# itailang/SampleNet

Measured on AMD Instinct MI355X. Metric: point-clouds/sec fwd+bwd, Bx1024->64 soft-proj+Chamfer, higher is better.
Workload: dtype f32; 1 GPU; BASELINE configs[1]: SampleNet sampler train step (fwd + simplification/projection losses + bwd), B=32 per GPU, 1024->64 points, K=8, bottleneck 128; no optimizer step; batch_per_gpu=32, global_batch=32, n_in=1024, n_out=64, group_size=8, parallelism=dp1, rccl_ranks=0, grad_allreduce=none, execution=whole step replayed as one hipGraph

## Files before the change

samplenet_amd/csrc/geometry_ops.hip:

```cpp
#include <algorithm>
#include <cstdlib>
#include <cstring>

#include "sn_common.h"
#include "step_tail.h"

#pragma clang fp contract(off)

namespace sn {

struct sn_xyz3 {
    float x, y, z;
};

constexpr int kMaxPrefixes = 16;

struct ImplicitGrad {
    const float *gL;
    const int *argmax_t, *argmax_s;
    float ct, cmax_t, cs, cmax_s;
    float gscale = 1.f;
};

__global__ void __launch_bounds__(256) chamfer_bwd_kernel(int nt, int ns, const float *__restrict__ T,
                                                          const float *__restrict__ S,
                                                          const float *__restrict__ gT,
                                                          const int *__restrict__ idxT,
                                                          const float *__restrict__ gS,
                                                          const int *__restrict__ idxS, float *__restrict__ gradT,
                                                          int own_first, ImplicitGrad ig, int t_layout)
{
    const int lane = threadIdx.x & 63;
    const int wave = __builtin_amdgcn_readfirstlane(threadIdx.x >> 6);
    const int nwaves = blockDim.x >> 6;
    const int b = blockIdx.x;
    T += (size_t)b * nt * 3, S += (size_t)b * ns * 3;
    idxT += (size_t)b * nt, idxS += (size_t)b * ns;
    const bool implicit = ig.gL != nullptr;
    float gLv = 0.f;
    int amt = -1, ams = -1;
    if (implicit) {
        gLv = *ig.gL * ig.gscale;
        if (ig.argmax_t) amt = ig.argmax_t[b];
        if (ig.argmax_s) ams = ig.argmax_s[b];
    } else {
        gT += (size_t)b * nt, gS += (size_t)b * ns;
    }
    gradT += (size_t)b * nt * 3;
    for (int j = blockIdx.y * nwaves + wave; j < nt; j += gridDim.y * nwaves) {
        const int o0 = t_layout ? j : j * 3, os = t_layout ? nt : 1;
        const float tx = T[o0], ty = T[o0 + os], tz = T[o0 + 2 * os];
        const int j2 = idxT[j];
        const float g = (implicit ? gLv * (ig.ct + (j == amt ? ig.cmax_t : 0.f)) : gT[j]) * 2;
        const float ox = g * (tx - S[j2 * 3 + 0]);
        const float oy = g * (ty - S[j2 * 3 + 1]);
        const float oz = g * (tz - S[j2 * 3 + 2]);
        float ax = 0.f, ay = 0.f, az = 0.f;
        if (own_first) ax += ox, ay += oy, az += oz;
        for (int l0 = 0; l0 < ns; l0 += 64 * 8) {
            int is[8];
#pragma unroll
            for (int q = 0; q < 8; ++q) {
                const int l = l0 + q * 64 + lane;
                is[q] = idxS[l < ns ? l : 0];
            }
#pragma unroll
            for (int q = 0; q < 8; ++q) {
                const int l = l0 + q * 64 + lane;
                sn_u64 mask = __ballot(l < ns && is[q] == j);
                while (mask) {
                    const int ll = l0 + q * 64 + __builtin_ctzll(mask);
                    mask &= mask - 1;
                    const float gg = (implicit ? gLv * (ig.cs + (ll == ams ? ig.cmax_s : 0.f)) : gS[ll]) * 2;
                    ax -= gg * (S[ll * 3 + 0] - tx);
                    ay -= gg * (S[ll * 3 + 1] - ty);
                    az -= gg * (S[ll * 3 + 2] - tz);
                }
            }
        }
        if (!own_first) ax += ox, ay += oy, az += oz;
        if (lane < 3) gradT[o0 + lane * os] = lane == 0 ? ax : (lane == 1 ? ay : az);
    }
}

template <int PPL>
__global__ void __launch_bounds__(256) chamfer_bwd_reg_kernel(int nt, int ns, const float *__restrict__ T,
                                                              const float *__restrict__ S,
                                                              const float *__restrict__ gT,
                                                              const int *__restrict__ idxT,
                                                              const float *__restrict__ gS,
                                                              const int *__restrict__ idxS, float *__restrict__ gradT,
                                                              int own_first, ImplicitGrad ig, int t_layout)
{
    const int lane = threadIdx.x & 63;
    const int wave = __builtin_amdgcn_readfirstlane(threadIdx.x >> 6);
    const int nwaves = blockDim.x >> 6;
    const int b = blockIdx.x;
    T += (size_t)b * nt * 3, S += (size_t)b * ns * 3;
    idxT += (size_t)b * nt, idxS += (size_t)b * ns;
    const bool implicit = ig.gL != nullptr;
    float gLv = 0.f;
    int amt = -1, ams = -1;
    if (implicit) {
        gLv = *ig.gL * ig.gscale;
        if (ig.argmax_t) amt = ig.argmax_t[b];
        if (ig.argmax_s) ams = ig.argmax_s[b];
    } else {
        gT += (size_t)b * nt, gS += (size_t)b * ns;
    }
    gradT += (size_t)b * nt * 3;

    float sx[PPL], sy[PPL], sz[PPL], gg[PPL];
    int is[PPL];
#pragma unroll
    for (int i = 0; i < PPL; ++i) {
        const int l = i * 64 + lane;
        const int lc = l < ns ? l : 0;
        const sn_xyz3 sv = *reinterpret_cast<const sn_xyz3 *>(S + (size_t)lc * 3);
        sx[i] = sv.x, sy[i] = sv.y, sz[i] = sv.z;
        is[i] = l < ns ? idxS[lc] : -1;
        gg[i] = (implicit ? gLv * (ig.cs + (l == ams ? ig.cmax_s : 0.f)) : gS[lc]) * 2;
    }
    for (int j = blockIdx.y * nwaves + wave; j < nt; j += gridDim.y * nwaves) {
        const int o0 = t_layout ? j : j * 3, os = t_layout ? nt : 1;
        const float tx = T[o0], ty = T[o0 + os], tz = T[o0 + 2 * os];
        const int j2 = idxT[j];
        const float g = (implicit ? gLv * (ig.ct + (j == amt ? ig.cmax_t : 0.f)) : gT[j]) * 2;
        const float ox = g * (tx - S[j2 * 3 + 0]);
        const float oy = g * (ty - S[j2 * 3 + 1]);
        const float oz = g * (tz - S[j2 * 3 + 2]);
        float ax = 0.f, ay = 0.f, az = 0.f;
        if (own_first) ax += ox, ay += oy, az += oz;
#pragma unroll
        for (int i = 0; i < PPL; ++i) {
            sn_u64 mask = __ballot(is[i] == j);
            if (mask) {
                const float cx = gg[i] * (sx[i] - tx), cy = gg[i] * (sy[i] - ty), cz = gg[i] * (sz[i] - tz);
                while (mask) {
                    const int t = __builtin_ctzll(mask);
                    mask &= mask - 1;
                    ax -= readlane_f(cx, t);
                    ay -= readlane_f(cy, t);
                    az -= readlane_f(cz, t);
                }
            }
        }
        if (!own_first) ax += ox, ay += oy, az += oz;
        if (lane < 3) gradT[o0 + lane * os] = lane == 0 ? ax : (lane == 1 ? ay : az);
    }
}

static const int kChamferBwdGroups = 1024;

static void launch_chamfer_bwd(int b, int ysplit, int nt, int ns, const float *T, const float *S, const float *gT,
                               const int *idxT, const float *gS, const int *idxS, float *gradT, int own_first,
                               const ImplicitGrad &ig, hipStream_t st, int t_layout = 0)
{
    const dim3 grid(b, ysplit), block(256);
#define SN_CB(PPL_) \
    hipLaunchKernelGGL(chamfer_bwd_reg_kernel<PPL_>, grid, block, 0, st, nt, ns, T, S, gT, idxT, gS, idxS, gradT, own_first, ig, t_layout)
    if (ns <= 64) SN_CB(1);
    else if (ns <= 256) SN_CB(4);
    else if (ns <= 1024) SN_CB(16);
    else if (ns <= 2048) SN_CB(32);
    else
        hipLaunchKernelGGL(chamfer_bwd_kernel, grid, block, 0, st, nt, ns, T, S, gT, idxT, gS, idxS, gradT, own_first, ig, t_layout);
#undef SN_CB
}

struct SoftBwdArgs {
    const float *P;
    const float *Q;
    const int *idx;
    const float *temperature;
    float min_sigma;
    int p_layout, q_layout;
    int n, m, k;
    const float *grad_proj;
    int gproj_layout;
    const float *weights_in;
    const float *grad_weights;
    float *grad_Q;
    int gq_layout;
    float *grad_P;
    float *gp_contrib;
    float *grad_sigma_partial;
    const float *gconst;
    float gconst_div;
    int accumulate_q;
};

struct SoftQuery {
    float qx, qy, qz;
    int id;
    float gx, gy, gz;
    float go0, go1, go2;
};

__device__ __forceinline__ float dpp_row_shr1(float x)
{
    return __int_as_float(__builtin_amdgcn_update_dpp(0, __float_as_int(x), 0x111, 0xf, 0xf, true));
}
__device__ __forceinline__ float dpp_row_shr1_self(float x)
{
    return __int_as_float(__builtin_amdgcn_update_dpp(__float_as_int(x), __float_as_int(x), 0x111, 0xf, 0xf, false));
}

__device__ __forceinline__ void soft_bwd_load_index(const SoftBwdArgs &a, int b, int j, int lane, const float *__restrict__ Qb,
                                                    SoftQuery &q)
{
    const int m = a.m, K = a.k;
    q.qx = Qb[pt_off(a.q_layout, m, j, 0)];
    q.qy = Qb[pt_off(a.q_layout, m, j, 1)];
    q.qz = Qb[pt_off(a.q_layout, m, j, 2)];
    const int sub = K <= 16 ? (lane & 15) : lane;
    q.id = sub < K ? a.idx[((size_t)b * m + j) * K + sub] : 0;
    q.go0 = q.go1 = q.go2 = 0.f;
    if (a.grad_proj) {
        const float *gp = a.grad_proj + (size_t)b * 3 * m;
        q.go0 = gp[pt_off(a.gproj_layout, m, j, 0)];
        q.go1 = gp[pt_off(a.gproj_layout, m, j, 1)];
        q.go2 = gp[pt_off(a.gproj_layout, m, j, 2)];
    }
}

__device__ __forceinline__ void soft_bwd_load_points(const SoftBwdArgs &a, int lane, const float *__restrict__ Pb, SoftQuery &q)
{
    const int n = a.n, K = a.k;
    const int sub = K <= 16 ? (lane & 15) : lane;
    q.gx = q.gy = q.gz = 0.f;
    if (sub < K) {
        q.gx = Pb[pt_off(a.p_layout, n, q.id, 0)];
        q.gy = Pb[pt_off(a.p_layout, n, q.id, 1)];
        q.gz = Pb[pt_off(a.p_layout, n, q.id, 2)];
    }
}

template <bool FUSED>
__device__ __forceinline__ void soft_bwd_math(const SoftBwdArgs &a, int b, int j, int lane, float sigma, const SoftQuery &q,
                                              float &aqx_o, float &aqy_o, float &aqz_o, float &asg_o)
{
    const int n = a.n, m = a.m, K = a.k;
    const bool rows = K <= 16;
    const int sub = rows ? (lane & 15) : lane;
    const bool act = sub < K;
    const int id = q.id;
    const float gx = q.gx, gy = q.gy, gz = q.gz;
    const float dx = gx - q.qx, dy = gy - q.qy, dz = gz - q.qz;
    const float d = (dx * dx + dy * dy) + dz * dz;
    const float s = act ? -(d / sigma) : -INFINITY;
    float mx, den;
    if (rows) {
        mx = s;
        for (int t = 1; t < K; ++t) mx = fmaxf(s, dpp_row_shr1_self(mx));
        mx = readlane_f(mx, K - 1);
    } else {
        mx = readlane_f(s, 0);
        for (int t = 1; t < K; ++t) mx = fmaxf(mx, readlane_f(s, t));
    }
    const float e = act ? expf(s - mx) : 0.f;
    if (rows) {
        den = e;
        for (int t = 1; t < K; ++t) den = e + dpp_row_shr1(den);
        den = readlane_f(den, K - 1);
    } else {
        den = 0.f;
        for (int t = 0; t < K; ++t) den += readlane_f(e, t);
    }
    const float w = e / den;

    float gw;
    float go0 = 0.f, go1 = 0.f, go2 = 0.f;
    if (FUSED) {
        if (a.grad_proj) {
            go0 = q.go0, go1 = q.go1, go2 = q.go2;
        } else {
            go0 = go1 = go2 = *a.gconst / a.gconst_div;
        }
        gw = (go0 * gx + go1 * gy) + go2 * gz;
    } else {
        gw = act ? a.grad_weights[((size_t)b * m + j) * K + sub] : 0.f;
    }
    float dot;
    if (rows) {
        const float wg = w * gw;
        dot = wg;
        for (int t = 1; t < K; ++t) dot = wg + dpp_row_shr1(dot);
        dot = readlane_f(dot, K - 1);
    } else {
        dot = 0.f;
        for (int t = 0; t < K; ++t) dot += readlane_f(w, t) * readlane_f(gw, t);
    }
    const float gs = act ? w * (gw - dot) : 0.f;
    const float gd = -gs / sigma;
    const float cx = 2.0f * gd * dx, cy = 2.0f * gd * dy, cz = 2.0f * gd * dz;
    const float sg = act ? gs * d / (sigma * sigma) : 0.f;
    float aqx = 0.f, aqy = 0.f, aqz = 0.f, asg = 0.f;
    if (rows) {
        const int row = lane >> 4;
// ... 124 lines not shown

__global__ void __launch_bounds__(256) weighted_gather_bwd_kernel(int c, int n, int m, int K,
                                                                  const float *__restrict__ X,
                                                                  const int *__restrict__ idx,
                                                                  const float *__restrict__ w,
                                                                  const float *__restrict__ go,
                                                                  float *__restrict__ gw, float *__restrict__ gX,
                                                                  float *__restrict__ contrib = nullptr)
{
    const int b = blockIdx.y;
    const size_t e = (size_t)blockIdx.x * blockDim.x + threadIdx.x;
    if (e >= (size_t)m * K) return;
    const int j = (int)(e / K);
    const int id = idx[(size_t)b * m * K + e];
    const float wt = w[(size_t)b * m * K + e];
    float acc = 0.f;
    for (int ch = 0; ch < c; ++ch) {
        const float g = go[((size_t)b * c + ch) * m + j];
        acc += g * X[((size_t)b * c + ch) * n + id];
        if (contrib) contrib[((size_t)b * c + ch) * m * K + e] = g * wt;
        else if (gX) atomicAdd(&gX[((size_t)b * c + ch) * n + id], g * wt);
    }
    if (gw) gw[(size_t)b * m * K + e] = acc;
}

__global__ void __launch_bounds__(256) group_point_kernel(int n, int c, int m, int ns, const float *__restrict__ points,
                                                          const int *__restrict__ idx, float *__restrict__ out)
{
    const int b = blockIdx.y;
    const size_t tot = (size_t)m * ns * c;
    for (size_t e = (size_t)blockIdx.x * blockDim.x + threadIdx.x; e < tot; e += (size_t)gridDim.x * blockDim.x) {
        const int l = (int)(e % c);
        const size_t jk = e / c;
        const int ii = idx[(size_t)b * m * ns + jk];
        out[(size_t)b * tot + e] = points[((size_t)b * n + ii) * c + l];
    }
}

template <bool CHANNEL_MAJOR>
__global__ void __launch_bounds__(256) index_add_ordered_kernel(int n, int c, int ne, const int *__restrict__ idx,
                                                                const float *__restrict__ src, float *__restrict__ dst)
{
    const int b = blockIdx.y, lane = threadIdx.x & 63;
    const int row0 = blockIdx.x * 256 + (threadIdx.x & ~63);
    const int row = row0 + lane;
    const bool live = row < n;
    idx += (size_t)b * ne;
    src += (size_t)b * ne * c;
    dst += (size_t)b * n * c;
    auto d = [&](int l) -> float & { return dst[CHANNEL_MAJOR ? (size_t)l * n + row : (size_t)row * c + l]; };
    if (live)
        for (int l = 0; l < c; ++l) d(l) = 0.f;
    for (int e0 = 0; e0 < ne; e0 += 64) {
        const int mine = e0 + lane < ne ? idx[e0 + lane] : -1;
        sn_u64 hits = __ballot((unsigned)(mine - row0) < 64u);
        while (hits) {
            const int t = __builtin_ctzll(hits);
            hits &= hits - 1;
            const int id = __builtin_amdgcn_readlane(mine, t), e = e0 + t;
            if (live && id == row)
                for (int l = 0; l < c; ++l) d(l) += src[CHANNEL_MAJOR ? (size_t)l * ne + e : (size_t)e * c + l];
        }
    }
}

constexpr long long kIndexAddOrderedWork = 1ll << 26;
template <bool CHANNEL_MAJOR>
__global__ void __launch_bounds__(256) index_add_atomic_kernel(int n, int c, long long ne, const int *__restrict__ idx,
                                                               const float *__restrict__ src, float *__restrict__ dst)
{
    const int b = blockIdx.y;
    idx += (size_t)b * ne;
    src += (size_t)b * ne * c;
    dst += (size_t)b * n * c;
    const size_t tot = (size_t)ne * c;
    for (size_t t = (size_t)blockIdx.x * blockDim.x + threadIdx.x; t < tot; t += (size_t)gridDim.x * blockDim.x) {
        const size_t e = CHANNEL_MAJOR ? t % (size_t)ne : t / c;
        const int l = (int)(CHANNEL_MAJOR ? t / (size_t)ne : t % c);
        const int row = idx[e];
        if ((unsigned)row < (unsigned)n) atomicAdd(&dst[CHANNEL_MAJOR ? (size_t)l * n + row : (size_t)row * c + l], src[t]);
    }
}

__global__ void __launch_bounds__(256) grouping_operation_kernel(int c, int n, int m, int ns,
                                                                 const float *__restrict__ feat,
                                                                 const int *__restrict__ idx, float *__restrict__ out)
{
    const int b = blockIdx.y;
    const size_t mk = (size_t)m * ns, tot = (size_t)c * mk;
    for (size_t e = (size_t)blockIdx.x * blockDim.x + threadIdx.x; e < tot; e += (size_t)gridDim.x * blockDim.x) {
        const int ch = (int)(e / mk);
        const size_t jk = e % mk;
        const int ii = idx[(size_t)b * mk + jk];
        out[(size_t)b * tot + e] = feat[((size_t)b * c + ch) * n + ii];
    }
}

static inline unsigned grid_for(size_t tot, int block = 256, unsigned cap = 4096)
{
    size_t g = (tot + block - 1) / block;
    return (unsigned)(g < 1 ? 1 : (g > cap ? cap : g));
}

}

using namespace sn;

struct StepLossFinal {
    int B, M, N, nproj;
    float w, alpha, lmbda, min_sigma;
    const float *part;
    const float *temperature;
    float *loss;
};

__device__ __forceinline__ void step_loss_final(const StepLossFinal &f, int t)
{
    float s1 = 0.f, mx = 0.f, s2 = 0.f, sp = 0.f;
    for (int b = t; b < f.B; b += 64) s1 += f.part[b * 4], mx += f.part[b * 4 + 1], s2 += f.part[b * 4 + 2], sp += f.part[b * 4 + 3];
    const float T = *f.temperature;
#pragma unroll
    for (int o = 32; o > 0; o >>= 1) {
        s1 += __shfl_xor(s1, o);
        mx += __shfl_xor(mx, o);
        s2 += __shfl_xor(s2, o);
        sp += __shfl_xor(sp, o);
    }
    if (t != 0) return;
    const float c12 = s1 / ((float)f.B * (float)f.M), cmax = mx / (float)f.B, c21 = s2 / ((float)f.B * (float)f.N);
    const float lsimp = c12 + cmax + f.w * c21;
    f.loss[0] = f.alpha * lsimp + f.lmbda * sn_sigma(T, f.min_sigma) + sp / ((float)f.B * (float)f.nproj);
    f.loss[1] = lsimp;
}

struct StepLossFold {
    int G;
    const sn_u64 *keys;
    const sn_u64 *qmax;
    float *dpsum;
};


#ifdef SN_CS_TIMELINE
__device__ unsigned long long g_cs_tl[8192 * 16];
#define CS_TL(slot)                                                                                              \
    do {                                                                                                         \
        if (threadIdx.x == 0) g_cs_tl[((blockIdx.y * gridDim.x + blockIdx.x) & 8191) * 16 + (slot)] = wall_clock64(); \
    } while (0)
#if SN_CS_TIMELINE >= 2
#define CS_TL_DRAIN() asm volatile("s_waitcnt vmcnt(0) lgkmcnt(0)" ::: "memory")
#else
#define CS_TL_DRAIN()
#endif
#else
#define CS_TL(slot)
#define CS_TL_DRAIN()
#endif

template <int PPL>
__global__ void __launch_bounds__(256) chamfer_soft_bwd_kernel(int nt, int ns, const float *__restrict__ T,
                                                               const float *__restrict__ S, const int *__restrict__ idxT,
                                                               const int *__restrict__ idxS, float *__restrict__ gradT,
                                                               ImplicitGrad ig, SoftBwdArgs sa, StepLossFinal fin,
                                                               StepLossFold fold)
{
    __shared__ float s_part[4];
    __shared__ int s_ip[PPL * 64];
    __shared__ float s_red[3][4];
    __shared__ int s_am;
    const int lane = threadIdx.x & 63;
    const int wave = __builtin_amdgcn_readfirstlane(threadIdx.x >> 6);
    const int nwaves = blockDim.x >> 6;
    const int b = blockIdx.x;
    CS_TL(0);
    kernarg_warm_for<24, int, int, const float *, const float *, const int *, const int *, float *, ImplicitGrad, SoftBwdArgs,
                     StepLossFinal, StepLossFold>();
    const int nsplit = fin.loss ? (int)gridDim.y - 1 : (int)gridDim.y;
    if ((int)blockIdx.y == nsplit) {
        if (b == 0 && wave == 0) step_loss_final(fin, lane);
        return;
    }
    T += (size_t)b * nt * 3, S += (size_t)b * ns * 3;
    idxT += (size_t)b * nt;
    if (idxS) idxS += (size_t)b * ns;
    gradT += (size_t)b * nt * 3;
    float sx[PPL], sy[PPL], sz[PPL], gg[PPL];
    int is[PPL];
#pragma unroll
    for (int i = 0; i < PPL; ++i) {
        const int l = i * 64 + lane;
        const int lc = l < ns ? l : 0;
        const sn_xyz3 sv = *reinterpret_cast<const sn_xyz3 *>(S + (size_t)lc * 3);
        sx[i] = sv.x, sy[i] = sv.y, sz[i] = sv.z;
    }
    const float gLv = *ig.gL * ig.gscale;
    const float Tm = *sa.temperature;
    const float sigma = sn_sigma(Tm, sa.min_sigma);
    const int jfirst = blockIdx.y * nwaves + wave, jstep = nsplit * nwaves;
    float tx = 0.f, ty = 0.f, tz = 0.f, ox = 0.f, oy = 0.f, oz = 0.f;
    int j2 = 0;
    SoftQuery sq{};
    auto load_query = [&](int j) {
        tx = T[j], ty = T[j + nt], tz = T[j + 2 * nt];
        j2 = idxT[j];
        soft_bwd_load_index(sa, b, j, lane, T, sq);
    };
    auto load_dependent = [&]() {
        ox = S[j2 * 3 + 0], oy = S[j2 * 3 + 1], oz = S[j2 * 3 + 2];
        soft_bwd_load_points(sa, lane, S, sq);
    };
    if (jfirst < nt) load_query(jfirst);
    CS_TL_DRAIN();
    CS_TL(8);

    if (fold.keys) {
        sn_u64 kv[PPL * 64 / 256 > 0 ? PPL * 64 / 256 : 1];
#pragma unroll
        for (int r = 0; r < (PPL * 64 + 255) / 256; ++r) {
            const int n = threadIdx.x + r * 256;
            kv[r] = fold.keys[(size_t)b * ns + (n < ns ? n : ns - 1)];
        }
        sn_u64 mk = 0;
        if (wave == 0) {
            for (int g = lane; g < fold.G; g += 64) {
                const sn_u64 v = fold.qmax[(size_t)b * fold.G + g];
                mk = v > mk ? v : mk;
            }
        }
#if defined(SN_CS_TIMELINE) && SN_CS_TIMELINE >= 2
        CS_TL_DRAIN();
        CS_TL(11);
#endif
        if (jfirst < nt) load_dependent();
        CS_TL_DRAIN();
        CS_TL(9);
        float sdp = 0.f;
#pragma unroll
        for (int r = 0; r < (PPL * 64 + 255) / 256; ++r) {
            const int n = threadIdx.x + r * 256;
            if (n < ns) {
                const sn_u64 k = ~kv[r];
                s_ip[n] = key_index(k);
                sdp += key_dist(k);
            }
        }
        if (blockIdx.y == 0) {
#pragma unroll
            for (int o = 32; o > 0; o >>= 1) sdp += __shfl_xor(sdp, o);
            if (lane == 0) s_red[2][wave] = sdp;
        }
        if (wave == 0) {
#pragma unroll
            for (int o = 32; o > 0; o >>= 1) {
                const unsigned hi = __shfl_xor((unsigned)(mk >> 32), o), lo = __shfl_xor((unsigned)mk, o);
                const sn_u64 v = ((sn_u64)hi << 32) | lo;
                mk = v > mk ? v : mk;
            }
            if (lane == 0) s_am = (int)(0xFFFFFFFFu - (unsigned)mk);
        }
        CS_TL(10);
        __syncthreads();
        if (blockIdx.y == 0 && threadIdx.x == 0) fold.dpsum[b] = (s_red[2][0] + s_red[2][1]) + (s_red[2][2] + s_red[2][3]);
    } else if (jfirst < nt) {
        load_dependent();
    }
    CS_TL(1);
    const int amt = fold.keys ? s_am : (ig.argmax_t ? ig.argmax_t[b] : -1), ams = ig.argmax_s ? ig.argmax_s[b] : -1;
    float gsig = 0.f;
#pragma unroll
    for (int i = 0; i < PPL; ++i) {
        const int l = i * 64 + lane;
        const int lc = l < ns ? l : 0;
        is[i] = l < ns ? (fold.keys ? s_ip[lc] : idxS[lc]) : -1;
        gg[i] = gLv * (ig.cs + (l == ams ? ig.cmax_s : 0.f)) * 2;
    }
    CS_TL_DRAIN();
    CS_TL(2);

    for (int j = jfirst; j < nt; j += jstep) {
        if (j != jfirst) {
            load_query(j);
            load_dependent();
        }
        const float g = gLv * (ig.ct + (j == amt ? ig.cmax_t : 0.f)) * 2;
        float ax = g * (tx - ox), ay = g * (ty - oy), az = g * (tz - oz);
        if (j == (int)blockIdx.y * nwaves) { CS_TL_DRAIN(); CS_TL(3); }
#pragma unroll
        for (int i = 0; i < PPL; ++i) {
            sn_u64 mask = __ballot(is[i] == j);
            if (mask) {
                const float cx = gg[i] * (sx[i] - tx), cy = gg[i] * (sy[i] - ty), cz = gg[i] * (sz[i] - tz);
                while (mask) {
                    const int t = __builtin_ctzll(mask);
                    mask &= mask - 1;
                    ax -= readlane_f(cx, t);
                    ay -= readlane_f(cy, t);
                    az -= readlane_f(cz, t);
                }
            }
        }
        if (j == (int)blockIdx.y * nwaves) CS_TL(4);
        float qx, qy, qz, asg;
        soft_bwd_math<true>(sa, b, j, lane, sigma, sq, qx, qy, qz, asg);
        if (j == (int)blockIdx.y * nwaves) CS_TL(5);
        gsig += asg;
        if (lane < 3) gradT[j + lane * nt] = lane == 0 ? ax + qx : (lane == 1 ? ay + qy : az + qz);
    }
    if (lane == 0) s_part[wave] = gsig;
    __syncthreads();
    if (threadIdx.x == 0) {
        float tot = 0.f;
        for (int w2 = 0; w2 < nwaves; ++w2) tot += s_part[w2];
        sa.grad_sigma_partial[(size_t)b * nsplit + blockIdx.y] = tot;
    }
    CS_TL_DRAIN();
    CS_TL(6);
}

extern "C" int sn_soft_bwd_splits(int b, int m)
{
    return std::max(1, std::min((m + 3) / 4, (kChamferBwdGroups + b - 1) / std::max(b, 1)));
}

extern "C" int sn_chamfer_backward(int b, int n, const float *xyz1, int m, const float *xyz2,
                                   const float *grad_dist1, const int *idx1, const float *grad_dist2,
                                   const int *idx2, float *grad_xyz1, float *grad_xyz2, sn_stream_t stream)
{
    SN_REQUIRE(b >= 0 && n >= 0 && m >= 0, "negative size");
    if (b == 0 || n == 0 || m == 0) return 0;
    SN_REQUIRE(xyz1 && xyz2 && grad_dist1 && grad_dist2 && idx1 && idx2, "null input");
    hipStream_t st = (hipStream_t)stream;
    auto ysplit = [&](int nt) { return std::max(1, std::min((nt + 3) / 4, (kChamferBwdGroups + b - 1) / b)); };
    const ImplicitGrad none{};
    if (grad_xyz1) launch_chamfer_bwd(b, ysplit(n), n, m, xyz1, xyz2, grad_dist1, idx1, grad_dist2, idx2, grad_xyz1, 1, none, st);
    if (grad_xyz2) launch_chamfer_bwd(b, ysplit(m), m, n, xyz2, xyz1, grad_dist2, idx2, grad_dist1, idx1, grad_xyz2, 0, none, st);
    SN_LAUNCH_CHECK();
    return 0;
}

__global__ void __launch_bounds__(256) simp_loss_partial_kernel(int n1, int n2, const float *__restrict__ d1,
                                                                const float *__restrict__ d2, float *__restrict__ part,
                                                                int *__restrict__ argmax1)
{
    __shared__ float r0[256], r1[256], r2[256];
    __shared__ int ri[256];
    const int b = blockIdx.x, t = threadIdx.x;
    float s1 = 0.f, mx = -INFINITY, s2 = 0.f;
    int am = 0;
    for (int j = t; j < n1; j += 256) {
        const float v = d1[(size_t)b * n1 + j];
        s1 += v;
        if (v > mx) mx = v, am = j;
    }
    for (int j = t; j < n2; j += 256) s2 += d2[(size_t)b * n2 + j];
    r0[t] = s1, r1[t] = mx, r2[t] = s2, ri[t] = am;
    for (int s = 128; s > 0; s >>= 1) {
        __syncthreads();
        if (t < s) {
            r0[t] += r0[t + s];
            r2[t] += r2[t + s];
            if (r1[t + s] > r1[t] || (r1[t + s] == r1[t] && ri[t + s] < ri[t])) r1[t] = r1[t + s], ri[t] = ri[t + s];
        }
    }
    if (t == 0) {
        part[b * 3 + 0] = r0[0], part[b * 3 + 1] = r1[0], part[b * 3 + 2] = r2[0];
        argmax1[b] = ri[0];
    }
}

template <bool WITH_MAX>
__global__ void __launch_bounds__(64) simp_loss_final_kernel(int B, int n1, int n2, float w, const float *__restrict__ part,
                                                             float *__restrict__ loss)
{
    if (threadIdx.x != 0) return;
    float s1 = 0.f, mx = 0.f, s2 = 0.f;
    for (int b = 0; b < B; ++b) s1 += part[b * 3], mx += part[b * 3 + 1], s2 += part[b * 3 + 2];
    const float c12 = s1 / ((float)B * (float)n1), cmax = mx / (float)B, c21 = s2 / ((float)B * (float)n2);
    loss[0] = WITH_MAX ? c12 + cmax + w * c21 : c12 + w * c21;
}

extern "C" int sn_simplification_loss_forward(int B, int n1, int n2, const float *dist1, const float *dist2, float weight,
                                              float *partial, int *argmax1, float *loss, sn_stream_t stream)
{
    SN_REQUIRE(B >= 1 && n1 >= 1 && n2 >= 1, "bad size");
    SN_REQUIRE(dist1 && dist2 && partial && argmax1 && loss, "null pointer");
    hipStream_t st = (hipStream_t)stream;
    hipLaunchKernelGGL(simp_loss_partial_kernel, dim3(B), dim3(256), 0, st, n1, n2, dist1, dist2, partial, argmax1);
    hipLaunchKernelGGL(simp_loss_final_kernel<true>, dim3(1), dim3(64), 0, st, B, n1, n2, weight, partial, loss);
    SN_LAUNCH_CHECK();
    return 0;
}

extern "C" int sn_simplification_loss_backward(int B, int n1, const float *xyz1, int n2, const float *xyz2, const int *idx1,
                                               const int *idx2, const int *argmax1, float weight, const float *grad_loss,
                                               float *grad_xyz1, float *grad_xyz2, int layout1, sn_stream_t stream)
{
    SN_REQUIRE(layout1 == 0 || layout1 == 1, "layout1 must be 0 (B,n1,3) or 1 (B,3,n1)");
    SN_REQUIRE(layout1 == 0 || !grad_xyz2, "grad_xyz2 needs xyz1 in (B,n1,3) layout");
    SN_REQUIRE(B >= 1 && n1 >= 1 && n2 >= 1, "bad size");
    SN_REQUIRE(xyz1 && xyz2 && idx1 && idx2 && argmax1 && grad_loss, "null pointer");
    hipStream_t st = (hipStream_t)stream;
    auto ysplit = [&](int nt) { return std::max(1, std::min((nt + 3) / 4, (kChamferBwdGroups + B - 1) / B)); };
    const float c1 = 1.0f / ((float)B * (float)n1), cm = 1.0f / (float)B, c2 = weight / ((float)B * (float)n2);
    if (grad_xyz1) {
        ImplicitGrad ig{grad_loss, argmax1, nullptr, c1, cm, c2, 0.f};
        launch_chamfer_bwd(B, ysplit(n1), n1, n2, xyz1, xyz2, nullptr, idx1, nullptr, idx2, grad_xyz1, 1, ig, st, layout1);
    }
    if (grad_xyz2) {
        ImplicitGrad ig{grad_loss, nullptr, argmax1, c2, 0.f, c1, cm};
        launch_chamfer_bwd(B, ysplit(n2), n2, n1, xyz2, xyz1, nullptr, idx2, nullptr, idx1, grad_xyz2, 0, ig, st);
    }
    SN_LAUNCH_CHECK();
    return 0;
}

extern "C" int sn_chamfer_mean_loss_forward(int B, int n1, int n2, const float *dist1, const float *dist2, float *partial,
                                            int *argmax1, float *loss, sn_stream_t stream)
{
    SN_REQUIRE(B >= 1 && n1 >= 1 && n2 >= 1, "bad size");
    SN_REQUIRE(dist1 && dist2 && partial && argmax1 && loss, "null pointer");
    hipStream_t st = (hipStream_t)stream;
    hipLaunchKernelGGL(simp_loss_partial_kernel, dim3(B), dim3(256), 0, st, n1, n2, dist1, dist2, partial, argmax1);
    hipLaunchKernelGGL(simp_loss_final_kernel<false>, dim3(1), dim3(64), 0, st, B, n1, n2, 1.0f, partial, loss);
    SN_LAUNCH_CHECK();
    return 0;
}

extern "C" int sn_chamfer_mean_loss_backward(int B, int n1, const float *xyz1, int n2, const float *xyz2, const int *idx1,
                                             const int *idx2, const float *grad_loss, float *grad_xyz1, float *grad_xyz2,
                                             sn_stream_t stream)
{
    SN_REQUIRE(B >= 1 && n1 >= 1 && n2 >= 1, "bad size");
    SN_REQUIRE(xyz1 && xyz2 && idx1 && idx2 && grad_loss, "null pointer");
    hipStream_t st = (hipStream_t)stream;
    auto ysplit = [&](int nt) { return std::max(1, std::min((nt + 3) / 4, (kChamferBwdGroups + B - 1) / B)); };
    const float c1 = 1.0f / ((float)B * (float)n1), c2 = 1.0f / ((float)B * (float)n2);
    if (grad_xyz1) {
        ImplicitGrad ig{grad_loss, nullptr, nullptr, c1, 0.f, c2, 0.f};
        launch_chamfer_bwd(B, ysplit(n1), n1, n2, xyz1, xyz2, nullptr, idx1, nullptr, idx2, grad_xyz1, 1, ig, st);
    }
    if (grad_xyz2) {
        ImplicitGrad ig{grad_loss, nullptr, nullptr, c2, 0.f, c1, 0.f};
        launch_chamfer_bwd(B, ysplit(n2), n2, n1, xyz2, xyz1, nullptr, idx2, nullptr, idx1, grad_xyz2, 0, ig, st);
    }
    SN_LAUNCH_CHECK();
    return 0;
}

struct GroupSizes {
    int n;
    int nv[kMaxPrefixes];
};
__global__ void __launch_bounds__(256) chamfer_mean_grouped_partial_kernel(int n1, int n2, int group, GroupSizes gs,
                                                                           const float *__restrict__ d1, const float *__restrict__ d2,
                                                                           float *__restrict__ part)
{
    __shared__ float r0[256], r2[256];
    const int b = blockIdx.x, t = threadIdx.x;
    const int nv = gs.nv[b / group];
    float s1 = 0.f, s2 = 0.f;
    for (int j = t; j < nv; j += 256) s1 += d1[(size_t)b * n1 + j];
    for (int j = t; j < n2; j += 256) s2 += d2[(size_t)b * n2 + j];
    r0[t] = s1, r2[t] = s2;
    for (int s = 128; s > 0; s >>= 1) {
        __syncthreads();
        if (t < s) r0[t] += r0[t + s], r2[t] += r2[t + s];
    }
    if (t == 0) part[b * 2] = r0[0], part[b * 2 + 1] = r2[0];
}
__global__ void __launch_bounds__(64) chamfer_mean_grouped_final_kernel(int n2, int group, GroupSizes gs, const float *__restrict__ part,
                                                                        float *__restrict__ loss)
{
    const int e = threadIdx.x;
    if (e >= gs.n) return;
    float s1 = 0.f, s2 = 0.f;
    for (int b = e * group; b < (e + 1) * group; ++b) s1 += part[b * 2], s2 += part[b * 2 + 1];
    const float c12 = s1 / ((float)group * (float)gs.nv[e]), c21 = s2 / ((float)group * (float)n2);
    loss[e] = c12 + 1.0f * c21;
}

static int group_sizes(const char *who, int R, int n1, int group, int nev, const int *nvalid, GroupSizes &gs)
{
    SN_REQUIRE_AS(who, group >= 1 && nev >= 1 && nev <= kMaxPrefixes && R == nev * group && nvalid, "R = nev * group, at most 16 evaluations");
    gs.n = nev;
    for (int e = 0; e < nev; ++e) {
        SN_REQUIRE_AS(who, nvalid[e] >= 1 && nvalid[e] <= n1, "valid points outside [1, n1]");
        gs.nv[e] = nvalid[e];
    }
    return 0;
}

extern "C" int sn_chamfer_mean_loss_forward_grouped(int R, int n1, int n2, int group, int nev, const int *nvalid, const float *dist1,
                                                    const float *dist2, float *partial, float *loss, sn_stream_t stream)
{
    SN_REQUIRE(R >= 1 && n1 >= 1 && n2 >= 1 && dist1 && dist2 && partial && loss, "bad argument");
    GroupSizes gs{};
    if (int rc = group_sizes(__func__, R, n1, group, nev, nvalid, gs)) return rc;
    hipStream_t st = (hipStream_t)stream;
    hipLaunchKernelGGL(chamfer_mean_grouped_partial_kernel, dim3(R), dim3(256), 0, st, n1, n2, group, gs, dist1, dist2, partial);
    hipLaunchKernelGGL(chamfer_mean_grouped_final_kernel, dim3(1), dim3(64), 0, st, n2, group, gs, partial, loss);
    SN_LAUNCH_CHECK();
    return 0;
}

struct GroupedGrad {
    const float *gL;
    int group;
    int t_valid;
    GroupSizes gs;
    float c_pad[kMaxPrefixes];
    float c_full;
};
template <int PPL>
__global__ void __launch_bounds__(256) chamfer_bwd_grouped_kernel(int nt, int ns, const float *__restrict__ T, const float *__restrict__ S,
                                                                  const int *__restrict__ idxT, const int *__restrict__ idxS,
                                                                  float *__restrict__ gradT, int own_first, GroupedGrad gg)
{
    const int lane = threadIdx.x & 63;
    const int wave = __builtin_amdgcn_readfirstlane(threadIdx.x >> 6);
    const int nwaves = blockDim.x >> 6;
    const int b = blockIdx.x, e = b / gg.group;
    T += (size_t)b * nt * 3, S += (size_t)b * ns * 3;
    idxT += (size_t)b * nt, idxS += (size_t)b * ns;
    gradT += (size_t)b * nt * 3;
    const float gLv = gg.gL[e] * 1.f;
    const float ct = gg.t_valid ? gg.c_pad[e] : gg.c_full, cs = gg.t_valid ? gg.c_full : gg.c_pad[e];
    const int ntv = gg.t_valid ? gg.gs.nv[e] : nt, nsv = gg.t_valid ? ns : gg.gs.nv[e];
    float sx[PPL], sy[PPL], sz[PPL], gs2[PPL];
    int is[PPL];
#pragma unroll
    for (int i = 0; i < PPL; ++i) {
        const int l = i * 64 + lane;
        const int lc = l < ns ? l : 0;
        const sn_xyz3 sv = *reinterpret_cast<const sn_xyz3 *>(S + (size_t)lc * 3);
        sx[i] = sv.x, sy[i] = sv.y, sz[i] = sv.z;
        is[i] = l < nsv ? idxS[lc] : -1;
        gs2[i] = (gLv * (cs + 0.f)) * 2;
    }
    for (int j = blockIdx.y * nwaves + wave; j < nt; j += gridDim.y * nwaves) {
        if (j >= ntv) {
            if (lane < 3) gradT[j * 3 + lane] = 0.f;
            continue;
        }
        const float tx = T[j * 3], ty = T[j * 3 + 1], tz = T[j * 3 + 2];
        const int j2 = idxT[j];
        const float g = (gLv * (ct + 0.f)) * 2;
        const float ox = g * (tx - S[j2 * 3 + 0]);
        const float oy = g * (ty - S[j2 * 3 + 1]);
        const float oz = g * (tz - S[j2 * 3 + 2]);
        float ax = 0.f, ay = 0.f, az = 0.f;
        if (own_first) ax += ox, ay += oy, az += oz;
#pragma unroll
        for (int i = 0; i < PPL; ++i) {
            sn_u64 mask = __ballot(is[i] == j);
            if (mask) {
                const float cx = gs2[i] * (sx[i] - tx), cy = gs2[i] * (sy[i] - ty), cz = gs2[i] * (sz[i] - tz);
                while (mask) {
                    const int t = __builtin_ctzll(mask);
                    mask &= mask - 1;
                    ax -= readlane_f(cx, t);
                    ay -= readlane_f(cy, t);
                    az -= readlane_f(cz, t);
                }
            }
        }
        if (!own_first) ax += ox, ay += oy, az += oz;
        if (lane < 3) gradT[j * 3 + lane] = lane == 0 ? ax : (lane == 1 ? ay : az);
    }
}

extern "C" int sn_chamfer_mean_loss_backward_grouped(int R, int n1, const float *xyz1, int n2, const float *xyz2, int group, int nev,
                                                     const int *nvalid, const int *idx1, const int *idx2, const float *grad_loss,
                                                     float *grad_xyz1, float *grad_xyz2, sn_stream_t stream)
{
    SN_REQUIRE(R >= 1 && n1 >= 1 && n2 >= 1 && n1 <= 2048 && n2 <= 2048, "bad size (at most 2048 points a side)");
    SN_REQUIRE(xyz1 && xyz2 && idx1 && idx2 && grad_loss, "null pointer");
    GroupedGrad gg{};
    if (int rc = group_sizes(__func__, R, n1, group, nev, nvalid, gg.gs)) return rc;
    gg.gL = grad_loss, gg.group = group;
    for (int e = 0; e < nev; ++e) gg.c_pad[e] = 1.0f / ((float)group * (float)nvalid[e]);
    gg.c_full = 1.0f / ((float)group * (float)n2);
    hipStream_t st = (hipStream_t)stream;
    auto ysplit = [&](int nt) { return std::max(1, std::min((nt + 3) / 4, (kChamferBwdGroups + R - 1) / R)); };
#define SN_CBG(PPL_, NT, NS, TT, SS, IT, IS, GT, OF)                                                                              \
    hipLaunchKernelGGL(chamfer_bwd_grouped_kernel<PPL_>, dim3(R, ysplit(NT)), dim3(256), 0, st, NT, NS, TT, SS, IT, IS, GT, OF, gg)
#define SN_CBG_ANY(NT, NS, TT, SS, IT, IS, GT, OF)           \
    do {                                                     \
        if (NS <= 64) SN_CBG(1, NT, NS, TT, SS, IT, IS, GT, OF);        \
        else if (NS <= 256) SN_CBG(4, NT, NS, TT, SS, IT, IS, GT, OF);  \
        else if (NS <= 1024) SN_CBG(16, NT, NS, TT, SS, IT, IS, GT, OF); \
        else SN_CBG(32, NT, NS, TT, SS, IT, IS, GT, OF);                \
    } while (0)
    if (grad_xyz1) {
        gg.t_valid = 1;
        SN_CBG_ANY(n1, n2, xyz1, xyz2, idx1, idx2, grad_xyz1, 1);
    }
    if (grad_xyz2) {
        gg.t_valid = 0;
        SN_CBG_ANY(n2, n1, xyz2, xyz1, idx2, idx1, grad_xyz2, 0);
    }
#undef SN_CBG_ANY
#undef SN_CBG
    SN_LAUNCH_CHECK();
    return 0;
}

__global__ void __launch_bounds__(256) pcrnet_head_fwd_kernel(int B, const float *__restrict__ y, float *__restrict__ twist,
                                                              float *__restrict__ quat, float *__restrict__ qnorm)
{
    __shared__ float red[256];
    float acc = 0.f;
    for (int b = threadIdx.x; b < B; b += 256) {
        const float *r = y + (size_t)b * 7;
        const float n2 = r[0] * r[0] + r[1] * r[1] + r[2] * r[2] + r[3] * r[3];
        const float inv = 1.0f / fmaxf(sqrtf(n2), 1e-12f);
        const float q0 = r[0] * inv, q1 = r[1] * inv, q2 = r[2] * inv, q3 = r[3] * inv;
        float *o = twist + (size_t)b * 7;
        o[0] = q0, o[1] = q1, o[2] = q2, o[3] = q3, o[4] = r[4], o[5] = r[5], o[6] = r[6];
        if (quat) quat[b * 4 + 0] = q0, quat[b * 4 + 1] = q1, quat[b * 4 + 2] = q2, quat[b * 4 + 3] = q3;
        acc += (n2 - 1.0f) * (n2 - 1.0f);
    }
    if (!qnorm) return;
    red[threadIdx.x] = acc;
    for (int s = 128; s > 0; s >>= 1) {
        __syncthreads();
        if (threadIdx.x < s) red[threadIdx.x] += red[threadIdx.x + s];
    }
    if (threadIdx.x == 0) qnorm[0] = red[0] / (float)B;
}

__global__ void __launch_bounds__(256) pcrnet_head_bwd_kernel(int B, const float *__restrict__ y, const float *__restrict__ g_twist,
                                                              const float *__restrict__ g_quat, const float *__restrict__ g_qnorm,
                                                              float *__restrict__ g_y)
{
    const float gq = g_qnorm ? g_qnorm[0] : 0.f;
    for (int b = threadIdx.x; b < B; b += 256) {
        const float *r = y + (size_t)b * 7;
        const float n2 = r[0] * r[0] + r[1] * r[1] + r[2] * r[2] + r[3] * r[3];
        const float nrm = sqrtf(n2);
        float *o = g_y + (size_t)b * 7;
        float gt[4] = {0.f, 0.f, 0.f, 0.f};
#pragma unroll
        for (int i = 0; i < 4; ++i) gt[i] = (g_twist ? g_twist[(size_t)b * 7 + i] : 0.f) + (g_quat ? g_quat[b * 4 + i] : 0.f);
        float gp[4];
        if (nrm > 1e-12f) {
            const float inv = 1.0f / nrm;
            const float q[4] = {r[0] * inv, r[1] * inv, r[2] * inv, r[3] * inv};
            const float dot = q[0] * gt[0] + q[1] * gt[1] + q[2] * gt[2] + q[3] * gt[3];
#pragma unroll
            for (int i = 0; i < 4; ++i) gp[i] = (gt[i] - q[i] * dot) * inv;
        } else {
#pragma unroll
            for (int i = 0; i < 4; ++i) gp[i] = gt[i] * 1e12f;
        }
#pragma unroll
        for (int i = 4; i < 7; ++i) o[i] = g_twist ? g_twist[(size_t)b * 7 + i] : 0.f;
        const float cq = gq * 4.0f * (n2 - 1.0f) / (float)B;
#pragma unroll
        for (int i = 0; i < 4; ++i) o[i] = gp[i] + cq * r[i];
    }
}

extern "C" int sn_pcrnet_head_forward(int B, const float *y, float *twist, float *quat, float *qnorm, sn_stream_t stream)
{
    SN_REQUIRE(B >= 1 && y && twist, "bad argument");
    hipLaunchKernelGGL(pcrnet_head_fwd_kernel, dim3(1), dim3(256), 0, (hipStream_t)stream, B, y, twist, quat, qnorm);
    SN_LAUNCH_CHECK();
    return 0;
}

extern "C" int sn_pcrnet_head_backward(int B, const float *y, const float *g_twist, const float *g_quat, const float *g_qnorm, float *g_y,
                                       sn_stream_t stream)
{
    SN_REQUIRE(B >= 1 && y && g_y, "bad argument");
    hipLaunchKernelGGL(pcrnet_head_bwd_kernel, dim3(1), dim3(256), 0, (hipStream_t)stream, B, y, g_twist, g_quat, g_qnorm, g_y);
    SN_LAUNCH_CHECK();
    return 0;
}

__global__ void __launch_bounds__(1024) sampler_loss_fwd_kernel(int nproj, const float *__restrict__ proj,
                                                                const float *__restrict__ lsimp,
                                                                const float *__restrict__ temperature, float alpha,
                                                                float lmbda, float min_sigma, float *__restrict__ loss)
{
    __shared__ float red[1024];
    float acc = 0.f;
    for (int i = threadIdx.x; i < nproj; i += 1024) acc += proj[i];
    red[threadIdx.x] = acc;
    for (int s = 512; s > 0; s >>= 1) {
        __syncthreads();
        if (threadIdx.x < s) red[threadIdx.x] += red[threadIdx.x + s];
    }
    if (threadIdx.x == 0) {
        const float T = *temperature;
        loss[0] = alpha * lsimp[0] + lmbda * sn_sigma(T, min_sigma) + red[0] / (float)nproj;
    }
}

__global__ void __launch_bounds__(256) sampler_loss_bwd_kernel(int nproj, const float *__restrict__ grad_loss,
                                                               const float *__restrict__ temperature, float alpha,
                                                               float lmbda, float min_sigma, float *__restrict__ grad_proj,
                                                               float *__restrict__ grad_lsimp, float *__restrict__ grad_T)
{
    const float g = grad_loss[0];
    const float gp = g / (float)nproj;
    for (int i = blockIdx.x * blockDim.x + threadIdx.x; i < nproj; i += gridDim.x * blockDim.x) grad_proj[i] = gp;
    if (blockIdx.x == 0 && threadIdx.x == 0) {
        grad_lsimp[0] = alpha * g;
        const float T = *temperature, t2 = T * T;
        const float w = t2 > min_sigma ? 1.f : (t2 == min_sigma ? 0.5f : 0.f);
        grad_T[0] = lmbda * g * w * 2.0f * T;
    }
}

extern "C" int sn_sampler_loss_forward(int nproj, const float *proj, const float *lsimp, const float *temperature,
                                       float alpha, float lmbda, float min_sigma, float *loss, sn_stream_t stream)
{
    SN_REQUIRE(nproj >= 1 && proj && lsimp && temperature && loss, "bad argument");
// ... 1157 lines not shown
    float s1 = 0.f, mx = -INFINITY, s2 = 0.f;
    int am = 0;
    for (int j = t; j < n1; j += 256) {
        const float v = d1[j];
        s1 += v;
        if (v > mx) mx = v, am = j;
    }
    for (int j = t; j < N; j += 256) s2 += dd[j];
    r0[t] = s1, r1[t] = mx, r2[t] = s2, ri[t] = am;
    for (int s = 128; s > 0; s >>= 1) {
        __syncthreads();
        if (t < s) {
            r0[t] += r0[t + s];
            r2[t] += r2[t + s];
            if (r1[t + s] > r1[t] || (r1[t + s] == r1[t] && ri[t + s] < ri[t])) r1[t] = r1[t + s], ri[t] = ri[t + s];
        }
    }
    if (t == 0) {
        float *o = part + ((size_t)p * B + b) * 3;
        o[0] = r0[0], o[1] = r1[0], o[2] = r2[0];
        argmax1[p * B + b] = ri[0];
    }
}

__global__ void __launch_bounds__(64) prefix_simp_final_kernel(int B, int N, PrefixLoss pl, const float *__restrict__ part,
                                                               float *__restrict__ loss)
{
    __shared__ float term[kMaxPrefixes];
    const int p = threadIdx.x;
    if (p < pl.n) {
        const float *q = part + (size_t)p * B * 3;
        float s1 = 0.f, mx = 0.f, s2 = 0.f;
        for (int b = 0; b < B; ++b) s1 += q[b * 3], mx += q[b * 3 + 1], s2 += q[b * 3 + 2];
        const float c12 = s1 / ((float)B * (float)pl.size[p]), cmax = mx / (float)B, c21 = s2 / ((float)B * (float)N);
        term[p] = c12 + cmax + pl.w[p] * c21;
    }
    __syncthreads();
    if (p == 0) {
        float tot = term[0];
        for (int j = 1; j < pl.n; ++j) tot += term[j];
        loss[0] = tot;
    }
}

template <int PPL>
__global__ void __launch_bounds__(256) prefix_simp_bwd_kernel(int M, int N, PrefixLoss pl, const float *__restrict__ T,
                                                              const float *__restrict__ S, const int *__restrict__ iq,
                                                              const int *__restrict__ i2, const int *__restrict__ argmax1,
                                                              const float *__restrict__ gL, float *__restrict__ gradT)
{
    const int lane = threadIdx.x & 63;
    const int wave = __builtin_amdgcn_readfirstlane(threadIdx.x >> 6);
    const int nwaves = blockDim.x >> 6;
    const int b = blockIdx.x, B = gridDim.x;
    T += (size_t)b * M * 3, S += (size_t)b * N * 3, iq += (size_t)b * M, gradT += (size_t)b * M * 3;
    const float gLv = *gL;
    float sx[PPL], sy[PPL], sz[PPL];
#pragma unroll
    for (int i = 0; i < PPL; ++i) {
        const int l = i * 64 + lane;
        const sn_xyz3 sv = *reinterpret_cast<const sn_xyz3 *>(S + (size_t)(l < N ? l : 0) * 3);
        sx[i] = sv.x, sy[i] = sv.y, sz[i] = sv.z;
    }
    for (int j = blockIdx.y * nwaves + wave; j < M; j += gridDim.y * nwaves) {
        const float tx = T[j * 3], ty = T[j * 3 + 1], tz = T[j * 3 + 2];
        const int j2 = iq[j];
        const float dx = tx - S[j2 * 3 + 0], dy = ty - S[j2 * 3 + 1], dz = tz - S[j2 * 3 + 2];
        float gx = 0.f, gy = 0.f, gz = 0.f;
        for (int p = pl.n - 1; p >= 0; --p) {
            const int n1 = pl.size[p];
            if (j >= n1) continue;
            const float g = gLv * (pl.c1[p] + (j == argmax1[p * B + b] ? pl.cm : 0.f)) * 2;
            const float gg = gLv * (pl.c2[p] + 0.f) * 2;
            float ax = g * dx, ay = g * dy, az = g * dz;
            const int *is = i2 + ((size_t)p * B + b) * N;
#pragma unroll
            for (int i = 0; i < PPL; ++i) {
                const int l = i * 64 + lane;
                sn_u64 mask = __ballot(l < N && is[l < N ? l : 0] == j);
                if (mask) {
                    const float cx = gg * (sx[i] - tx), cy = gg * (sy[i] - ty), cz = gg * (sz[i] - tz);
                    while (mask) {
                        const int t = __builtin_ctzll(mask);
                        mask &= mask - 1;
                        ax -= readlane_f(cx, t);
                        ay -= readlane_f(cy, t);
                        az -= readlane_f(cz, t);
                    }
                }
            }
            gx += ax, gy += ay, gz += az;
        }
        if (lane < 3) gradT[j * 3 + lane] = lane == 0 ? gx : (lane == 1 ? gy : gz);
    }
}

static int prefix_loss_args(int B, int M, int N, int nterms, const int *sizes, const float *weights, PrefixLoss &pl)
{
    SN_REQUIRE(nterms >= 1 && nterms <= kMaxPrefixes && sizes && weights, "1..16 prefix terms");
    pl.n = nterms;
    for (int j = 0; j < nterms; ++j) {
        SN_REQUIRE(sizes[j] >= 1 && sizes[j] <= M, "prefix size outside [1, M]");
        pl.size[j] = sizes[j], pl.w[j] = weights[j];
        pl.c1[j] = 1.0f / ((float)B * (float)sizes[j]), pl.c2[j] = weights[j] / ((float)B * (float)N);
    }
    pl.cm = 1.0f / (float)B;
    return 0;
}

extern "C" int sn_prefix_simplification_loss_forward(int B, int M, int N, int nterms, const int *sizes, const float *weights,
                                                     const float *dq, const float *d2, float *partial, int *argmax1, float *loss,
                                                     sn_stream_t stream)
{
    SN_REQUIRE(B >= 1 && M >= 1 && N >= 1 && dq && d2 && partial && argmax1 && loss, "bad argument");
    PrefixLoss pl{};
    if (int rc = prefix_loss_args(B, M, N, nterms, sizes, weights, pl)) return rc;
    hipStream_t st = (hipStream_t)stream;
    hipLaunchKernelGGL(prefix_simp_partial_kernel, dim3(B, nterms), dim3(256), 0, st, M, N, pl, dq, d2, partial, argmax1);
    hipLaunchKernelGGL(prefix_simp_final_kernel, dim3(1), dim3(64), 0, st, B, N, pl, partial, loss);
    SN_LAUNCH_CHECK();
    return 0;
}

extern "C" int sn_prefix_simplification_loss_backward(int B, int M, int N, int nterms, const int *sizes, const float *weights,
                                                      const float *samp_pc, const float *ref_pc, const int *iq, const int *i2,
                                                      const int *argmax1, const float *grad_loss, float *grad_samp, sn_stream_t stream)
{
    SN_REQUIRE(B >= 1 && M >= 1 && N >= 1 && N <= 2048, "bad size (N <= 2048)");
    SN_REQUIRE(samp_pc && ref_pc && iq && i2 && argmax1 && grad_loss && grad_samp, "null pointer");
    PrefixLoss pl{};
    if (int rc = prefix_loss_args(B, M, N, nterms, sizes, weights, pl)) return rc;
    hipStream_t st = (hipStream_t)stream;
    const dim3 grid(B, std::max(1, std::min((M + 3) / 4, (kChamferBwdGroups + B - 1) / B))), block(256);
#define SN_PB(PPL_) \
    hipLaunchKernelGGL(prefix_simp_bwd_kernel<PPL_>, grid, block, 0, st, M, N, pl, samp_pc, ref_pc, iq, i2, argmax1, grad_loss, grad_samp)
    if (N <= 64) SN_PB(1);
    else if (N <= 256) SN_PB(4);
    else if (N <= 1024) SN_PB(16);
    else SN_PB(32);
#undef SN_PB
    SN_LAUNCH_CHECK();
    return 0;
}

#ifdef SN_CS_TIMELINE
extern "C" int sn_debug_chamfer_soft_bwd_timeline(void *host, int nblocks)
{
    if (nblocks < 0 || nblocks > 8192) return -1;
    if (hipDeviceSynchronize() != hipSuccess) return -2;
    if (hipMemcpyFromSymbol(host, HIP_SYMBOL(g_cs_tl), (size_t)nblocks * 16 * 8) != hipSuccess) return -3;
    static unsigned long long zeros[8192 * 16];
    return hipMemcpyToSymbol(HIP_SYMBOL(g_cs_tl), zeros, sizeof(zeros)) == hipSuccess ? 0 : -4;
}
#endif
```

Measured before the change: 183,800 point-clouds/s.

## Replace serial readlane owner accumulation with LDS compaction and DPP row reduction

In the Chamfer backward kernels, the per-target loop used to walk every owning source lane with a serial readlane chain for x, y and z. It now compacts the owner contributions into per-wave LDS lists with mbcnt prefix ranks. It then sums them with DPP row-rotate accumulation, 16 lanes per coordinate in parallel. This shortens the serial scalar dependency chain when a target has many owners, at the cost of LDS writes, fences, and overhead when owners are few. It also adds optional timing instrumentation that is compiled only under a debug macro.

```diff
diff --git a/samplenet_amd/csrc/geometry_ops.hip b/samplenet_amd/csrc/geometry_ops.hip
--- a/samplenet_amd/csrc/geometry_ops.hip
+++ b/samplenet_amd/csrc/geometry_ops.hip
@@ -83,6 +83,90 @@
     }
 }
 
+constexpr int kOwnerCap = 256;
+constexpr int kOwnerRow = kOwnerCap + 16;
+struct OwnerList {
+    float c[3][kOwnerRow];
+};
+
+__device__ __forceinline__ float dpp_row_ror1(float x)
+{
+    return __int_as_float(__builtin_amdgcn_update_dpp(0, __float_as_int(x), 0x121, 0xf, 0xf, true));
+}
+
+template <int PPL>
+__device__ __forceinline__ void owner_sum(OwnerList &L, int lane, int j, const int (&is)[PPL], const float (&gg)[PPL],
+                                          const float (&sx)[PPL], const float (&sy)[PPL], const float (&sz)[PPL], float tx,
+                                          float ty, float tz, float &ax, float &ay, float &az)
+{
+    const int row = lane >> 4, sub = lane & 15;
+    const float *col = &L.c[row < 3 ? row : 2][sub];
+    float acc = row == 0 ? ax : (row == 1 ? ay : az);
+    int at = 15;
+    auto drain = [&](int cnt) {
+        __builtin_amdgcn_fence(__ATOMIC_ACQ_REL, "wavefront");
+        float v = sub < cnt ? col[0] : 0.f;
+#pragma nounroll
+        for (int c0 = 0; c0 < cnt; c0 += 16) {
+            const int e = c0 + 16 + sub;
+            const float vn = e < cnt ? col[c0 + 16] : 0.f;
+            const int rem = cnt - c0;
+            if (rem >= 16) {
+#pragma unroll
+                for (int t = 0; t < 16; ++t) acc = dpp_row_ror1(acc) - v;
+            } else {
+#pragma nounroll
+                for (int t = 0; t < rem; t += 4) {
+                    acc = dpp_row_ror1(acc) - v;
+                    acc = dpp_row_ror1(acc) - v;
+                    acc = dpp_row_ror1(acc) - v;
+                    acc = dpp_row_ror1(acc) - v;
+                }
+                at = ((rem + 3) & ~3) - 1;
+            }
+            v = vn;
+        }
+        __builtin_amdgcn_fence(__ATOMIC_ACQ_REL, "wavefront");
+        __builtin_amdgcn_s_waitcnt(0xc07f);
+    };
+    int total = 0;
+#pragma unroll
+    for (int i = 0; i < PPL; ++i) {
+        const bool own = is[i] == j;
+        const sn_u64 mask = __ballot(own);
+        if (mask) {
+            const float cx = gg[i] * (sx[i] - tx), cy = gg[i] * (sy[i] - ty), cz = gg[i] * (sz[i] - tz);
+            const unsigned r = total + __builtin_amdgcn_mbcnt_hi((unsigned)(mask >> 32), __builtin_amdgcn_mbcnt_lo((unsigned)mask, 0u));
+            const unsigned rc = r < (unsigned)kOwnerCap ? r : (unsigned)kOwnerCap;
+            if (own) L.c[0][rc] = cx, L.c[1][rc] = cy, L.c[2][rc] = cz;
+            total += __builtin_popcountll(mask);
+        }
+    }
+    drain(total < kOwnerCap ? total : kOwnerCap);
+#pragma nounroll
+    for (int base = kOwnerCap; base < total; base += kOwnerCap) {
+        j = __builtin_amdgcn_readfirstlane(j);
+        asm volatile("" : "+v"(tx), "+v"(ty), "+v"(tz), "+s"(j));
+        int n = 0;
+#pragma unroll
+        for (int i = 0; i < PPL; ++i) {
+            const bool own = is[i] == j;
+            const sn_u64 mask = __ballot(own);
+            if (mask) {
+                const int n0 = n;
+                n += __builtin_popcountll(mask);
+                if (n > base && n0 < base + kOwnerCap) {
+                    const float cx = gg[i] * (sx[i] - tx), cy = gg[i] * (sy[i] - ty), cz = gg[i] * (sz[i] - tz);
+                    const int r = n0 - base + (int)__builtin_amdgcn_mbcnt_hi((unsigned)(mask >> 32), __builtin_amdgcn_mbcnt_lo((unsigned)mask, 0u));
+                    if (own && (unsigned)r < (unsigned)kOwnerCap) L.c[0][r] = cx, L.c[1][r] = cy, L.c[2][r] = cz;
+                }
+            }
+        }
+        drain(total - base < kOwnerCap ? total - base : kOwnerCap);
+    }
+    ax = readlane_f(acc, at), ay = readlane_f(acc, 16 + at), az = readlane_f(acc, 32 + at);
+}
+
 template <int PPL>
 __global__ void __launch_bounds__(256) chamfer_bwd_reg_kernel(int nt, int ns, const float *__restrict__ T,
                                                               const float *__restrict__ S,
@@ -92,6 +176,7 @@
                                                               const int *__restrict__ idxS, float *__restrict__ gradT,
                                                               int own_first, ImplicitGrad ig, int t_layout)
 {
+    __shared__ OwnerList s_own[4];
     const int lane = threadIdx.x & 63;
     const int wave = __builtin_amdgcn_readfirstlane(threadIdx.x >> 6);
     const int nwaves = blockDim.x >> 6;
@@ -131,20 +216,7 @@
         const float oz = g * (tz - S[j2 * 3 + 2]);
         float ax = 0.f, ay = 0.f, az = 0.f;
         if (own_first) ax += ox, ay += oy, az += oz;
-#pragma unroll
-        for (int i = 0; i < PPL; ++i) {
-            sn_u64 mask = __ballot(is[i] == j);
-            if (mask) {
-                const float cx = gg[i] * (sx[i] - tx), cy = gg[i] * (sy[i] - ty), cz = gg[i] * (sz[i] - tz);
-                while (mask) {
-                    const int t = __builtin_ctzll(mask);
-                    mask &= mask - 1;
-                    ax -= readlane_f(cx, t);
-                    ay -= readlane_f(cy, t);
-                    az -= readlane_f(cz, t);
-                }
-            }
-        }
+        owner_sum<PPL>(s_own[wave], lane, j, is, gg, sx, sy, sz, tx, ty, tz, ax, ay, az);
         if (!own_first) ax += ox, ay += oy, az += oz;
         if (lane < 3) gradT[o0 + lane * os] = lane == 0 ? ax : (lane == 1 ? ay : az);
     }
@@ -575,9 +647,26 @@
 #else
 #define CS_TL_DRAIN()
 #endif
+__device__ unsigned g_cs_walk[8192 * 4];
+#define CS_WALK_BEGIN()                                              \
+    asm volatile("s_waitcnt vmcnt(0) lgkmcnt(0)" ::: "memory"); \
+    const unsigned long long walk_t0 = wall_clock64()
+#define CS_WALK_END(x, y, z)                                                                          \
+    do {                                                                                              \
+        asm volatile("; owner sum done" ::"v"(x), "v"(y), "v"(z) : "memory");                         \
+        const unsigned walk_dt = (unsigned)(wall_clock64() - walk_t0);                                \
+        walk_max = walk_dt > walk_max ? walk_dt : walk_max;                                           \
+    } while (0)
+#define CS_WALK_STORE()                                                                                                   \
+    do {                                                                                                                  \
+        if (lane == 0) g_cs_walk[((blockIdx.y * gridDim.x + blockIdx.x) & 8191) * 4 + wave] = walk_max + 1u;  \
+    } while (0)
 #else
 #define CS_TL(slot)
 #define CS_TL_DRAIN()
+#define CS_WALK_BEGIN()
+#define CS_WALK_END(x, y, z)
+#define CS_WALK_STORE()
 #endif
 
 template <int PPL>
@@ -591,6 +680,7 @@
     __shared__ int s_ip[PPL * 64];
     __shared__ float s_red[3][4];
     __shared__ int s_am;
+    __shared__ OwnerList s_own[4];
     const int lane = threadIdx.x & 63;
     const int wave = __builtin_amdgcn_readfirstlane(threadIdx.x >> 6);
     const int nwaves = blockDim.x >> 6;
@@ -690,6 +780,9 @@
     CS_TL(1);
     const int amt = fold.keys ? s_am : (ig.argmax_t ? ig.argmax_t[b] : -1), ams = ig.argmax_s ? ig.argmax_s[b] : -1;
     float gsig = 0.f;
+#ifdef SN_CS_TIMELINE
+    unsigned walk_max = 0;
+#endif
 #pragma unroll
     for (int i = 0; i < PPL; ++i) {
         const int l = i * 64 + lane;
@@ -708,20 +801,9 @@
         const float g = gLv * (ig.ct + (j == amt ? ig.cmax_t : 0.f)) * 2;
         float ax = g * (tx - ox), ay = g * (ty - oy), az = g * (tz - oz);
         if (j == (int)blockIdx.y * nwaves) { CS_TL_DRAIN(); CS_TL(3); }
-#pragma unroll
-        for (int i = 0; i < PPL; ++i) {
-            sn_u64 mask = __ballot(is[i] == j);
-            if (mask) {
-                const float cx = gg[i] * (sx[i] - tx), cy = gg[i] * (sy[i] - ty), cz = gg[i] * (sz[i] - tz);
-                while (mask) {
-                    const int t = __builtin_ctzll(mask);
-                    mask &= mask - 1;
-                    ax -= readlane_f(cx, t);
-                    ay -= readlane_f(cy, t);
-                    az -= readlane_f(cz, t);
-                }
-            }
-        }
+        CS_WALK_BEGIN();
+        owner_sum<PPL>(s_own[wave], lane, j, is, gg, sx, sy, sz, tx, ty, tz, ax, ay, az);
+        CS_WALK_END(ax, ay, az);
         if (j == (int)blockIdx.y * nwaves) CS_TL(4);
         float qx, qy, qz, asg;
         soft_bwd_math<true>(sa, b, j, lane, sigma, sq, qx, qy, qz, asg);
@@ -736,6 +818,7 @@
         for (int w2 = 0; w2 < nwaves; ++w2) tot += s_part[w2];
         sa.grad_sigma_partial[(size_t)b * nsplit + blockIdx.y] = tot;
     }
+    if (jfirst < nt) CS_WALK_STORE();
     CS_TL_DRAIN();
     CS_TL(6);
 }
@@ -939,6 +1022,7 @@
                                                                   const int *__restrict__ idxT, const int *__restrict__ idxS,
                                                                   float *__restrict__ gradT, int own_first, GroupedGrad gg)
 {
+    __shared__ OwnerList s_own[4];
     const int lane = threadIdx.x & 63;
     const int wave = __builtin_amdgcn_readfirstlane(threadIdx.x >> 6);
     const int nwaves = blockDim.x >> 6;
@@ -973,20 +1057,7 @@
         const float oz = g * (tz - S[j2 * 3 + 2]);
         float ax = 0.f, ay = 0.f, az = 0.f;
         if (own_first) ax += ox, ay += oy, az += oz;
-#pragma unroll
-        for (int i = 0; i < PPL; ++i) {
-            sn_u64 mask = __ballot(is[i] == j);
-            if (mask) {
-                const float cx = gs2[i] * (sx[i] - tx), cy = gs2[i] * (sy[i] - ty), cz = gs2[i] * (sz[i] - tz);
-                while (mask) {
-                    const int t = __builtin_ctzll(mask);
-                    mask &= mask - 1;
-                    ax -= readlane_f(cx, t);
-                    ay -= readlane_f(cy, t);
-                    az -= readlane_f(cz, t);
-                }
-            }
-        }
+        owner_sum<PPL>(s_own[wave], lane, j, is, gs2, sx, sy, sz, tx, ty, tz, ax, ay, az);
         if (!own_first) ax += ox, ay += oy, az += oz;
         if (lane < 3) gradT[j * 3 + lane] = lane == 0 ? ax : (lane == 1 ? ay : az);
     }
@@ -2450,4 +2521,12 @@
     static unsigned long long zeros[8192 * 16];
     return hipMemcpyToSymbol(HIP_SYMBOL(g_cs_tl), zeros, sizeof(zeros)) == hipSuccess ? 0 : -4;
 }
+extern "C" int sn_debug_chamfer_soft_bwd_walk(void *host, int nblocks)
+{
+    if (nblocks < 0 || nblocks > 8192) return -1;
+    if (hipDeviceSynchronize() != hipSuccess) return -2;
+    if (hipMemcpyFromSymbol(host, HIP_SYMBOL(g_cs_walk), (size_t)nblocks * 4 * 4) != hipSuccess) return -3;
+    static unsigned zeros[8192 * 4];
+    return hipMemcpyToSymbol(HIP_SYMBOL(g_cs_walk), zeros, sizeof(zeros)) == hipSuccess ? 0 : -4;
+}
 #endif
```

Result: faster. 186,000 point-clouds/s, median of 6 (+1.2%).
